# samiazirar/mvtracker

Hardware: AMD Instinct MI355X
Metric: query-points*frames/sec, 4-view 24-frame 512x512 @1024 queries (higher is better)
Workload: dtype bf16; 1 GPU; c3: 4-view synthetic 24-frame 512x512, 1024 queries, bf16 (configs[2], the metric's config); 4-view 24-frame 512x512, 1024 queries per GPU, corr K=16 x 4 levels, iters=4, 3 windows, random-init weights (seeded recipe); queries_total=1024, parallelism=query-shard x1, frame_store=bf16 rows

## Files before the change

### mvtracker_amd/csrc/conv_rows.hip

```cpp
#include <stdlib.h>

#include "common.h"

namespace {

typedef __bf16 bf16x8 __attribute__((ext_vector_type(8)));
typedef __bf16 bf16x4 __attribute__((ext_vector_type(4)));
typedef unsigned u32x4 __attribute__((ext_vector_type(4)));
typedef unsigned u32x2 __attribute__((ext_vector_type(2)));
typedef float f32x2 __attribute__((ext_vector_type(2)));
typedef short s16x2 __attribute__((ext_vector_type(2)));
typedef __bf16 bf16x2 __attribute__((ext_vector_type(2)));

#ifdef MVT_STAMPS
#ifndef MVT_STAMP_WG
#define MVT_STAMP_WG 2000
#endif
__device__ unsigned long long mvt_conv_stamp_buf[2 * 8 * 128];
#define CSTAMP(i)                                                                                                  \
  do {                                                                                                             \
    __builtin_amdgcn_sched_barrier(0);                                                                             \
    unsigned long long t_;                                                                                         \
    asm volatile("s_memtime %0\n\ts_waitcnt lgkmcnt(0)" : "=s"(t_)::"memory");                                     \
    __builtin_amdgcn_sched_barrier(0);                                                                             \
// ... 606 lines not shown

constexpr int SPR = 2 * TR + 5, SPC = 2 * TC + 6;
constexpr int SNP = SPR * SPC;
constexpr int SKW = 7 * 32;
constexpr int SLW = SKW + 8;

template <int TN, bool STAGED>
__global__ __launch_bounds__(256) void stem7x7_rows_bf16(RowsArgs p) {
  constexpr int TM = 2, BN = TN * 32;
  constexpr int NPL = (SNP + 255) / 256;
  constexpr int NWF = (BN * (SKW / 8) + 255) / 256;
  __shared__ __attribute__((aligned(16))) unsigned short Ps[SNP * 4];
  __shared__ __attribute__((aligned(16))) unsigned short Ws[BN * SLW];
  __shared__ float wst[TR * BN * 2];
  const int t = threadIdx.x;
  for (int i = t; i < TR * BN * 2; i += 256) wst[i] = 0.f;
  const int Ho = (p.H + 6 - 7) / 2 + 1, Wo = (p.W + 6 - 7) / 2 + 1;
  const int tiles_x = (Wo + TC - 1) / TC, tiles_y = (Ho + TR - 1) / TR;
  int b = blockIdx.x;
  const int tx = b % tiles_x; b /= tiles_x;
  const int ty = b % tiles_y;
  const long long img = b / tiles_y;
  const int y0 = ty * TR, x0 = tx * TC;
  const float* in = p.in + img * (long long)p.H * p.W * 4;
  const long long hw = (long long)p.H * p.W;
  long long plane0 = 0;
  if (p.rgb) {
    const long long gi = p.rgb_img0 + img;
    const long long tt = gi / p.rgb_V, vv = gi - tt * p.rgb_V;
    plane0 = ((vv * p.rgb_T + tt) * 3) * hw;
  }

  f32x4 rp[NPL];
#pragma unroll
  for (int i = 0; i < NPL; ++i) {
    const int f = t + 256 * i;
    const int py = f / SPC, px = f - py * SPC;
    const int gy = 2 * y0 - 3 + py, gx = 2 * x0 - 3 + px;
    const bool ok = f < SNP && (unsigned)gy < (unsigned)p.H && (unsigned)gx < (unsigned)p.W;
    const int cy = min(max(gy, 0), p.H - 1), cx = min(max(gx, 0), p.W - 1);
    f32x4 v;
    if (p.rgb) {
      const long long o = plane0 + (long long)cy * p.W + cx;
      float c0, c1, c2;
      if (p.rgb_u8) {
        const unsigned char* sp = static_cast<const unsigned char*>(p.rgb) + o;
        c0 = (float)sp[0]; c1 = (float)sp[hw]; c2 = (float)sp[2 * hw];
      } else {
        const float* sp = static_cast<const float*>(p.rgb) + o;
        c0 = sp[0]; c1 = sp[hw]; c2 = sp[2 * hw];
      }
      v = (f32x4){2.0f * (c0 / 255.0f) - 1.0f, 2.0f * (c1 / 255.0f) - 1.0f, 2.0f * (c2 / 255.0f) - 1.0f, 0.0f};
    } else {
      v = *reinterpret_cast<const f32x4*>(in + ((long long)cy * p.W + cx) * 4);
    }
    rp[i] = ok ? v : (f32x4){0.f, 0.f, 0.f, 0.f};
  }
  u32x4 rw[NWF];
#pragma unroll
  for (int i = 0; i < NWF; ++i) {
    const int u = t + 256 * i;
    const int n = u / (SKW / 8), part = u - n * (SKW / 8);
    rw[i] = *reinterpret_cast<const u32x4*>(p.w + (long long)min(n, p.Cout - 1) * p.ldw + part * 8);
    if (n >= p.Cout) rw[i] = (u32x4){0u, 0u, 0u, 0u};
  }
#pragma unroll
  for (int i = 0; i < NPL; ++i) {
    const int f = t + 256 * i;
    if (f < SNP) *reinterpret_cast<u32x2*>(&Ps[f * 4]) = __builtin_bit_cast(u32x2, __builtin_convertvector(rp[i], bf16x4));
  }
#pragma unroll
  for (int i = 0; i < NWF; ++i) {
    const int u = t + 256 * i;
    const int n = u / (SKW / 8), part = u - n * (SKW / 8);
    if (n < BN) *reinterpret_cast<u32x4*>(&Ws[n * SLW + part * 8]) = rw[i];
  }
  __syncthreads();

  const int lane = t & 63;
  const int wm = __builtin_amdgcn_readfirstlane(t >> 6);
  const int r = lane & 31, h = lane >> 5;
  const unsigned short* Pl = Ps + ((wm * TM * 2) * SPC + 2 * r + 2 * h) * 4;
  const unsigned short* Wl = Ws + r * SLW + h * 8;
  f32x16 acc[TM][TN];
#pragma unroll
  for (int i = 0; i < TM; ++i)
#pragma unroll
    for (int j = 0; j < TN; ++j)
#pragma unroll
      for (int e = 0; e < 16; ++e) acc[i][j][e] = 0.f;
#pragma unroll
  for (int kh = 0; kh < 7; ++kh) {
#pragma unroll
    for (int ks = 0; ks < 2; ++ks) {
      bf16x8 a[TM], bb[TN];
#pragma unroll
      for (int i = 0; i < TM; ++i) a[i] = __builtin_bit_cast(bf16x8, *reinterpret_cast<const u32x4*>(Pl + ((2 * i + kh) * SPC + 4 * ks) * 4));
#pragma unroll
      for (int j = 0; j < TN; ++j) bb[j] = __builtin_bit_cast(bf16x8, *reinterpret_cast<const u32x4*>(Wl + j * 32 * SLW + kh * 32 + ks * 16));
#pragma unroll
      for (int i = 0; i < TM; ++i)
#pragma unroll
        for (int j = 0; j < TN; ++j) acc[i][j] = __builtin_amdgcn_mfma_f32_32x32x16_bf16(a[i], bb[j], acc[i][j], 0, 0, 0);
    }
  }

  __syncthreads();
  static_assert(4 * stage_elems<TN>() <= BN * SLW, "staging tiles fit the weight buffer");
  epilogue_rows<TM, TN, true, STAGED>(acc, p, img, Ho, Wo, y0 + wm * TM, x0, 0, tiles_x, tx, lane, Ws + wm * stage_elems<TN>(), wst, wm * TM);
  if (p.out_part) {
    __syncthreads();
    write_tile_stats<TR, BN>(p, wst, img, ty * tiles_x + tx, 0, t);
  }
}


constexpr int BG_BN = 256;
constexpr int BG_PC = TC + 2;
constexpr int BG_PSLOTS = (TR + 2) * BG_PC;
constexpr int BG_PINSTR = 24;
constexpr int BG_PBYTES = BG_PINSTR * 1024;
constexpr int BG_PROW = BG_PC * 64;
constexpr int BG_WBYTES = 3 * BG_BN * 64;
constexpr int BG_WST = TR * BG_BN * 2 * 4;
constexpr int BG_LDS = 2 * BG_PBYTES + 2 * BG_WBYTES;
static_assert(BG_PSLOTS * 64 <= BG_PBYTES, "patch slots fit the buffer");
static_assert(BG_WBYTES / 1024 == 6 * 8, "six weight DMA wave-instructions per wave and stage");
static_assert(BG_LDS <= 160 * 1024 && BG_WST <= 2 * BG_WBYTES, "one workgroup per CU");
static_assert(8 * stage_elems<2>() * 2 <= 2 * BG_PBYTES, "the epilogue's staging tiles reuse the patch buffers");

__device__ __attribute__((aligned(64))) unsigned mvt_conv_zero_page[16];

typedef __attribute__((address_space(3))) void* lds_void_ptr;
typedef const __attribute__((address_space(1))) void* gbl_void_ptr;

__device__ __forceinline__ void dma16(const void* src, unsigned char* lds_dst_uniform) {
  const unsigned dst = __builtin_amdgcn_readfirstlane((unsigned)(uintptr_t)(lds_void_ptr)lds_dst_uniform);
  unsigned keep;
  asm volatile("s_mov_b32 %0, m0\n\ts_mov_b32 m0, %2\n\ts_nop 0\n\tglobal_load_lds_dwordx4 %1, off\n\ts_mov_b32 m0, %0"
               : "=&s"(keep)
               : "v"(src), "s"(dst)
               : "memory");
}

__global__ __launch_bounds__(512, 2) void conv3x3_big_bf16(RowsArgs p) {
  constexpr int TM = 4, TN = 2;
  __shared__ __attribute__((aligned(1024))) unsigned char lds[BG_LDS];
  unsigned char* const Pb = lds;
  unsigned char* const Wb = lds + 2 * BG_PBYTES;
  float* const wst = reinterpret_cast<float*>(Wb);

  const int t = threadIdx.x, lane = t & 63;
  const int wave = __builtin_amdgcn_readfirstlane(t >> 6);
  const int wm = wave & 1, wn = wave >> 1;
  const int r = lane & 31, h = lane >> 5;
  const int Ho = p.H, Wo = p.W;
  const int tiles_x = (Wo + TC - 1) / TC, tiles_y = (Ho + TR - 1) / TR;
  const int tiles_n = p.Cout / BG_BN;
  int b;
  {
    const unsigned nwg = gridDim.x, q = nwg / 8, rr = nwg % 8, xcd = blockIdx.x % 8;
    b = (int)((xcd < rr ? xcd * (q + 1) : rr * (q + 1) + (xcd - rr) * q) + blockIdx.x / 8);
  }
  const int tn = b % tiles_n; b /= tiles_n;
  const int tx = b % tiles_x; b /= tiles_x;
  const int ty = b % tiles_y;
  const long long img = b / tiles_y;
  const int y0 = ty * TR, x0 = tx * TC, n0 = tn * BG_BN;
  const unsigned char* const in_img = reinterpret_cast<const unsigned char*>(p.in) + img * (long long)p.H * p.W * p.Cin * 2;
  const unsigned char* const wbase = reinterpret_cast<const unsigned char*>(p.w);
  const unsigned char* const zero = reinterpret_cast<const unsigned char*>(mvt_conv_zero_page);

  int poff[3];
#pragma unroll
  for (int i = 0; i < 3; ++i) {
    const int P = (wave + 8 * i) * 64 + lane;
    const int slot = P >> 2, py = slot / BG_PC, px = slot - py * BG_PC;
    const int q = (P & 3) ^ ((px >> 2) & 3);
    const int gy = y0 - 1 + py, gx = x0 - 1 + px;
    const bool ok = slot < BG_PSLOTS && (unsigned)gy < (unsigned)p.H && (unsigned)gx < (unsigned)p.W;
    poff[i] = ok ? ((gy * p.W + gx) * p.Cin + q * 8) * 2 : -1;
  }
  int woff[6];
#pragma unroll
  for (int i = 0; i < 6; ++i) {
    const int R = (wave + 8 * i) * 16 + (lane >> 2);
    const int q = (lane & 3) ^ ((R >> 2) & 3);
    woff[i] = ((n0 + (R & 255)) * p.ldw + (R >> 8) * p.Cin + q * 8) * 2;
  }
  auto dma_weight = [&](int stage, int dst_stage, int i) {
    const int c = stage / 3, kh = stage - 3 * c;
    dma16(wbase + ((long long)kh * 3 * p.Cin + c * CK) * 2 + woff[i], Wb + (dst_stage & 1) * BG_WBYTES + wave * 1024 + i * 8192);
  };
  auto dma_patch1 = [&](int c, int dst_c, int i) {
    dma16(poff[i] >= 0 ? in_img + c * CK * 2 + poff[i] : zero, Pb + (dst_c & 1) * BG_PBYTES + wave * 1024 + i * 8192);
  };

  const int nchunk = p.Cin / CK;
#pragma unroll
  for (int i = 0; i < 3; ++i) dma_patch1(0, 0, i);
#pragma unroll
  for (int i = 0; i < 6; ++i) dma_weight(0, 0, i);

  int pa[3][2], wl[2];
#pragma unroll
  for (int kw = 0; kw < 3; ++kw)
#pragma unroll
    for (int ks = 0; ks < 2; ++ks)
      pa[kw][ks] = (TM * wm * BG_PC + kw + r) * 64 + (((2 * ks + h) ^ (((kw + r) >> 2) & 3)) << 4);
#pragma unroll
  for (int ks = 0; ks < 2; ++ks) wl[ks] = (64 * wn + r) * 64 + (((2 * ks + h) ^ ((r >> 2) & 3)) << 4);

  f32x16 acc[TM][TN];
#pragma unroll
  for (int i = 0; i < TM; ++i)
#pragma unroll
    for (int j = 0; j < TN; ++j)
#pragma unroll
      for (int e = 0; e < 16; ++e) acc[i][j][e] = 0.f;

  bf16x8 a[2][TM], bb[2][TN];
  auto read_group = [&](int set, int g, int kh, const unsigned char* Pc, const unsigned char* Wc) {
    const int kw = g >> 1, ks = g & 1;
#pragma unroll
    for (int i = 0; i < TM; ++i)
      a[set][i] = __builtin_bit_cast(bf16x8, *reinterpret_cast<const u32x4*>(Pc + pa[kw][ks] + (i + kh) * BG_PROW));
#pragma unroll
    for (int j = 0; j < TN; ++j)
      bb[set][j] = __builtin_bit_cast(bf16x8, *reinterpret_cast<const u32x4*>(Wc + wl[ks] + kw * (BG_BN * 64) + j * 2048));
  };
  auto mfma_group = [&](int set) {
#pragma unroll
    for (int i = 0; i < TM; ++i)
#pragma unroll
      for (int j = 0; j < TN; ++j) acc[i][j] = __builtin_amdgcn_mfma_f32_32x32x16_bf16(a[set][i], bb[set][j], acc[i][j], 0, 0, 0);
  };
  CSTAMP(0);
#ifdef MVT_BIG_PRIO
  if (wave >= 4) __builtin_amdgcn_s_setprio(1);
#endif
  asm volatile("s_waitcnt vmcnt(0)" ::: "memory");
  __builtin_amdgcn_s_barrier();
  read_group(0, 0, 0, Pb, Wb);
  for (int c = 0; c < nchunk; ++c) {
    const unsigned char* const Pc = Pb + (c & 1) * BG_PBYTES;
#pragma unroll
    for (int kh = 0; kh < 3; ++kh) {
      const int stage = 3 * c + kh;
      const int stage_n = stage + 1 < 3 * nchunk ? stage + 1 : stage, chunk_n = c + 1 < nchunk ? c + 1 : c;
      const unsigned char* const Wc = Wb + (stage & 1) * BG_WBYTES;
#pragma unroll
      for (int g = 0; g < 5; ++g) {
        read_group((g + 1) & 1, g + 1, kh, Pc, Wc);
#ifdef MVT_BIG_EARLY
        if (g == 0) {
#pragma unroll
          for (int i = 0; i < 6; ++i) dma_weight(stage_n, stage + 1, i);
        } else if (g == 1 && kh == 0) {
#pragma unroll
          for (int i = 0; i < 3; ++i) dma_patch1(chunk_n, c + 1, i);
        }
#else
        if (g < 3) {
          dma_weight(stage_n, stage + 1, 2 * g);
          dma_weight(stage_n, stage + 1, 2 * g + 1);
        } else if (kh == 0) {
          dma_patch1(chunk_n, c + 1, g == 3 ? 0 : 2);
          if (g == 3) dma_patch1(chunk_n, c + 1, 1);
        }
#endif
        __builtin_amdgcn_sched_barrier(0);
        mfma_group(g & 1);
        __builtin_amdgcn_sched_barrier(0);
        if (stage < 12) CSTAMP(1 + 10 * stage + g);
      }
      if (kh == 0) asm volatile("s_waitcnt vmcnt(3) lgkmcnt(0)" ::: "memory");
      else asm volatile("s_waitcnt vmcnt(0) lgkmcnt(0)" ::: "memory");
      if (stage < 12) CSTAMP(1 + 10 * stage + 5);
      __builtin_amdgcn_s_barrier();
      if (stage < 12) CSTAMP(1 + 10 * stage + 6);
      read_group(0, 0, kh == 2 ? 0 : kh + 1, kh == 2 ? Pb + ((c + 1) & 1) * BG_PBYTES : Pc, Wb + ((stage + 1) & 1) * BG_WBYTES);
      __builtin_amdgcn_sched_barrier(0);
      mfma_group(1);
      __builtin_amdgcn_sched_barrier(0);
      if (stage < 12) CSTAMP(1 + 10 * stage + 7);
    }
  }
  CSTAMP(124);
  asm volatile("s_waitcnt vmcnt(0)" ::: "memory");
  __builtin_amdgcn_s_barrier();
  for (int i = lane; i < TM * 64 * 2; i += 64) wst[((wm * TM + (i >> 7)) * BG_BN + wn * 64) * 2 + (i & 127)] = 0.f;

  epilogue_rows<TM, TN, false, true, BG_BN>(acc, p, img, Ho, Wo, y0 + wm * TM, x0, n0 + wn * 64, tiles_x, tx, lane,
                                             reinterpret_cast<unsigned short*>(Pb) + wave * stage_elems<TN>(), wst + wn * 64 * 2, wm * TM);
  CSTAMP(125);
  if (p.out_part) {
    __syncthreads();
    write_tile_stats<TR, BG_BN>(p, wst, img, ty * tiles_x + tx, n0, t);
  }
  CSTAMP(126);
}


}

#ifdef MVT_STAMPS
extern "C" int mvt_debug_read_conv_stamps(unsigned long long* host) {
  return hipMemcpyFromSymbol(host, HIP_SYMBOL(mvt_conv_stamp_buf), sizeof(unsigned long long) * 2 * 8 * 128) == hipSuccess ? MVT_OK : MVT_ERR_HIP_BASE;
}
extern "C" int mvt_debug_clear_conv_stamps() {
  static unsigned long long z[2 * 8 * 128];
  return hipMemcpyToSymbol(HIP_SYMBOL(mvt_conv_stamp_buf), z, sizeof(z)) == hipSuccess ? MVT_OK : MVT_ERR_HIP_BASE;
}
#endif

static int rows_nw8() {
  static const int v = getenv("MVT_ROWS_NW8") ? atoi(getenv("MVT_ROWS_NW8")) : 0;
  return v;
}
__attribute__((visibility("hidden"))) int mvt_detail_conv_rows_tile_rows(int ksize, int stride, int Ho) {
  if (ksize == 3 && stride == 1) return (rows_nw8() == 1 && Ho % 16 == 0) ? 16 : (rows_nw8() == 2 ? 4 : 8);
  if (ksize == 3) return 4;
  if (ksize == 7) return TR;
  return 8;
}
__attribute__((visibility("hidden"))) int mvt_detail_conv_rows_slots(int Ho, int Wo, int tile_rows) {
  return (int)(mvt_cdiv(Ho, tile_rows) * mvt_cdiv(Wo, TC));
}

__attribute__((visibility("hidden"))) int mvt_detail_conv_rows(const void* in, const unsigned short* w, int ldw, const float* bias, void* out,
                                                               int n, int H, int W, int Cin, int Cout, int ksize, int stride, int ldo,
                                                               int io_flags, const float* in_stats, float* out_partial,
                                                               hipStream_t stream) {
  MVT_REQUIRE((ksize == 1 || ksize == 3) && (stride == 1 || stride == 2));
  MVT_REQUIRE((!in_stats || Cin <= MAXC) && Cin % CK == 0 && (long long)H * W * Cin < (1LL << 31) && (long long)Cout * ldw < (1LL << 31));
  MVT_REQUIRE((long long)(TC + 8) * ldo * 4 < (1LL << 31));
  const int pad = ksize == 3 ? 1 : 0;
  const int Ho = (H + 2 * pad - ksize) / stride + 1, Wo = (W + 2 * pad - ksize) / stride + 1;
  RowsArgs a{};
  a.in = (const float*)in; a.w = w; a.bias = bias; a.out = (float*)out; a.in_stats = in_stats; a.out_part = out_partial;
  a.H = H; a.W = W; a.Cin = Cin; a.Cout = Cout; a.ldw = ldw; a.ldo = ldo;
  a.slots = mvt_detail_conv_rows_slots(Ho, Wo, mvt_detail_conv_rows_tile_rows(ksize, stride, Ho));
  a.in_bf16 = io_flags & MVT_IO_IN_BF16 ? 1 : 0;
  a.out_bf16 = io_flags & MVT_IO_OUT_BF16 ? 1 : 0;
  const bool n96 = Cout % 64 != 0 && Cout % 96 == 0;
  const int bn = n96 ? 96 : 64;
  const bool st_ok = a.out_bf16 && Cout % 8 == 0 && ldo % 8 == 0 && ((uintptr_t)out & 15) == 0;
#define LAUNCH2(TM_, TN_, KS_, S_, NW_, INB_)                                                                                       \
  do {                                                                                                                             \
    constexpr bool fits = NW_ * stage_elems<TN_>() <= Geo<TM_, KS_, S_, NW_>::NSLOT * LDP;                                          \
    if (fits && st_ok) hipLaunchKernelGGL((conv_rows_bf16<TM_, TN_, KS_, S_, INB_, NW_, fits>), grid, dim3(64 * NW_), 0, stream, a); \
    else hipLaunchKernelGGL((conv_rows_bf16<TM_, TN_, KS_, S_, INB_, NW_, false>), grid, dim3(64 * NW_), 0, stream, a);            \
  } while (0)
#define LAUNCH(TM_, KS_, S_, NW_)                                                                                                   \
  do {                                                                                                                             \
    const long long tiles = (long long)n * mvt_cdiv(Ho, NW_ * TM_) * mvt_cdiv(Wo, TC) * mvt_cdiv(Cout, bn);                        \
    MVT_REQUIRE(tiles < (1LL << 31));                                                                                              \
    const dim3 grid((unsigned)tiles);                                                                                              \
    if (n96) {                                                                                                                     \
      if (a.in_bf16) LAUNCH2(TM_, 3, KS_, S_, NW_, true);                                                                          \
      else LAUNCH2(TM_, 3, KS_, S_, NW_, false);                                                                                   \
    } else {                                                                                                                       \
      if (a.in_bf16) LAUNCH2(TM_, 2, KS_, S_, NW_, true);                                                                          \
      else LAUNCH2(TM_, 2, KS_, S_, NW_, false);                                                                                   \
    }                                                                                                                              \
  } while (0)
  const int nw8 = rows_nw8();
  if (ksize == 3 && stride == 1 && !in_stats && !(io_flags & MVT_IO_SHORT_WG) && a.in_bf16 && st_ok && Cout % BG_BN == 0 && ((uintptr_t)in & 15) == 0 && Cin % 8 == 0 &&
      ldw % 8 == 0 && ((uintptr_t)w & 15) == 0 && (long long)Cout * ldw * 2 < (1LL << 31) && (long long)H * W * Cin * 2 < (1LL << 31)) {
    const char* e = getenv("MVT_CONV_BIG");
    if (!e || atoi(e) != 0) {
      const long long tiles = (long long)n * mvt_cdiv(Ho, TR) * mvt_cdiv(Wo, TC) * (Cout / BG_BN);
      MVT_REQUIRE(tiles < (1LL << 31));
      hipLaunchKernelGGL(conv3x3_big_bf16, dim3((unsigned)tiles), dim3(512), 0, stream, a);
      return mvt_launch_status();
    }
  }
  if (ksize == 3 && stride == 1 && nw8 == 1 && Ho % 16 == 0) LAUNCH(2, 3, 1, 8);
  else if (ksize == 3 && stride == 1 && nw8 == 2) LAUNCH(1, 3, 1, 4);
  else if (ksize == 3 && stride == 1) LAUNCH(2, 3, 1, 4);
  else if (ksize == 3) LAUNCH(1, 3, 2, 4);
  else if (stride == 1) LAUNCH(2, 1, 1, 4);
  else LAUNCH(2, 1, 2, 4);
#undef LAUNCH2
#undef LAUNCH
  return mvt_launch_status();
}

__attribute__((visibility("hidden"))) int mvt_detail_conv3x3s2_down(const void* in, const unsigned short* w3, int ldw3, const float* b3,
                                                                    const unsigned short* wd, int ldwd, const float* bd, void* out3,
                                                                    void* outd, int n, int H, int W, int Cin, int Cout, int ldo,
                                                                    float* part3, float* partd, hipStream_t stream) {
  MVT_REQUIRE(in && w3 && wd && out3 && outd && n > 0 && Cin % CK == 0 && Cout % 32 == 0 && Cout % 8 == 0 && ldo % 8 == 0 && ldo >= Cout);
  MVT_REQUIRE((long long)H * W * Cin < (1LL << 31) && (long long)Cout * ldw3 < (1LL << 31) && ldwd >= Cin && ldw3 >= 9 * Cin);
  MVT_REQUIRE(((uintptr_t)in & 15) == 0 && ((uintptr_t)out3 & 15) == 0 && ((uintptr_t)outd & 15) == 0 && ((uintptr_t)w3 & 15) == 0 &&
              ((uintptr_t)wd & 15) == 0 && ldw3 % 8 == 0 && ldwd % 8 == 0 && (!part3) == (!partd));
  const int Ho = (H + 2 - 3) / 2 + 1, Wo = (W + 2 - 3) / 2 + 1;
  RowsArgs a{};
  a.in = (const float*)in; a.w = w3; a.bias = b3; a.out = (float*)out3; a.in_stats = nullptr; a.out_part = part3;
  a.H = H; a.W = W; a.Cin = Cin; a.Cout = Cout; a.ldw = ldw3; a.ldo = ldo;
  a.slots = mvt_detail_conv_rows_slots(Ho, Wo, 4);
  a.in_bf16 = 1; a.out_bf16 = 1;
  a.w2 = wd; a.bias2 = bd; a.out2 = (float*)outd; a.out_part2 = partd; a.ldw2 = ldwd;
  const bool n96 = Cout % 64 != 0 && Cout % 96 == 0;
  const long long tiles = (long long)n * mvt_cdiv(Ho, 4) * mvt_cdiv(Wo, TC) * mvt_cdiv(Cout, n96 ? 96 : 64);
  MVT_REQUIRE(tiles < (1LL << 31));
  static_assert(4 * stage_elems<2>() <= Geo<1, 3, 2, 4>::NSLOT * LDP && 4 * stage_elems<3>() <= Geo<1, 3, 2, 4>::NSLOT * LDP, "staged epilogue");
  if (n96) hipLaunchKernelGGL((conv_rows_bf16<1, 3, 3, 2, true, 4, true, true>), dim3((unsigned)tiles), dim3(256), 0, stream, a);
  else hipLaunchKernelGGL((conv_rows_bf16<1, 2, 3, 2, true, 4, true, true>), dim3((unsigned)tiles), dim3(256), 0, stream, a);
  return mvt_launch_status();
}

__attribute__((visibility("hidden"))) int mvt_detail_stem7x7_rows_src(const float* in, const void* rgb, int rgb_u8, int rgb_V, int rgb_T,
                                                                      long long rgb_img0, const unsigned short* w, int ldw,
                                                                      const float* bias, void* out, int n, int H, int W, int Cout, int ldo,
                                                                      int io_flags, float* out_partial, hipStream_t stream);
__attribute__((visibility("hidden"))) int mvt_detail_stem7x7_rows(const float* in, const unsigned short* w, int ldw, const float* bias,
                                                                  void* out, int n, int H, int W, int Cout, int ldo, int io_flags,
                                                                  float* out_partial, hipStream_t stream) {
  return mvt_detail_stem7x7_rows_src(in, nullptr, 0, 0, 0, 0, w, ldw, bias, out, n, H, W, Cout, ldo, io_flags, out_partial, stream);
}
__attribute__((visibility("hidden"))) int mvt_detail_stem7x7_rows_src(const float* in, const void* rgb, int rgb_u8, int rgb_V, int rgb_T,
                                                                      long long rgb_img0, const unsigned short* w, int ldw,
                                                                      const float* bias, void* out, int n, int H, int W, int Cout, int ldo,
                                                                      int io_flags, float* out_partial, hipStream_t stream) {
  MVT_REQUIRE(Cout > 0 && Cout <= 64 && ldw >= SKW && (long long)H * W * 4 < (1LL << 31) && !(io_flags & MVT_IO_IN_BF16));
  MVT_REQUIRE((in != nullptr) != (rgb != nullptr));
  MVT_REQUIRE(!rgb || (rgb_V > 0 && rgb_T > 0 && rgb_img0 >= 0 && rgb_img0 + n <= (long long)rgb_V * rgb_T && (rgb_u8 == 0 || rgb_u8 == 1)));
  const int Ho = (H - 1) / 2 + 1, Wo = (W - 1) / 2 + 1;
  RowsArgs a{};
  a.rgb = rgb; a.rgb_u8 = rgb_u8; a.rgb_V = rgb_V; a.rgb_T = rgb_T; a.rgb_img0 = rgb_img0;
  a.in = in; a.w = w; a.bias = bias; a.out = (float*)out; a.in_stats = nullptr; a.out_part = out_partial;
  a.H = H; a.W = W; a.Cin = 4; a.Cout = Cout; a.ldw = ldw; a.ldo = ldo;
  a.slots = mvt_detail_conv_rows_slots(Ho, Wo, TR);
  a.in_bf16 = 0;
  a.out_bf16 = io_flags & MVT_IO_OUT_BF16 ? 1 : 0;
  const long long tiles = (long long)n * mvt_cdiv(Ho, TR) * mvt_cdiv(Wo, TC);
  MVT_REQUIRE(tiles < (1LL << 31) && (long long)(TC + 8) * ldo * 4 < (1LL << 31));
  const bool st_ok = a.out_bf16 && Cout % 8 == 0 && ldo % 8 == 0 && ((uintptr_t)out & 15) == 0;
  if (Cout <= 32) {
    if (st_ok) hipLaunchKernelGGL((stem7x7_rows_bf16<1, true>), dim3((unsigned)tiles), dim3(256), 0, stream, a);
    else hipLaunchKernelGGL((stem7x7_rows_bf16<1, false>), dim3((unsigned)tiles), dim3(256), 0, stream, a);
  } else {
    if (st_ok) hipLaunchKernelGGL((stem7x7_rows_bf16<2, true>), dim3((unsigned)tiles), dim3(256), 0, stream, a);
    else hipLaunchKernelGGL((stem7x7_rows_bf16<2, false>), dim3((unsigned)tiles), dim3(256), 0, stream, a);
  }
  return mvt_launch_status();
}
```

Baseline: 1.020 million query-points*frames/s.

## Add four-workgroup-per-CU 3x3 conv kernel for normalized or small-channel rows

Adds a new 256-thread 3x3 stride-1 bf16 convolution kernel sized to fit four workgroups per CU in LDS. It fuses input normalization/ReLU from per-image stats into the patch store, register-prefetches the next weight row and patch chunk, and remaps block ids across XCDs. It is dispatched for cases the big kernel rejects (for example in_stats present) when there are enough tiles. It also stops caching the env var lookup, which adds a getenv per call.

```diff
diff --git a/mvtracker_amd/csrc/conv_rows.hip b/mvtracker_amd/csrc/conv_rows.hip
--- a/mvtracker_amd/csrc/conv_rows.hip
+++ b/mvtracker_amd/csrc/conv_rows.hip
@@ -932,6 +932,169 @@
 }
 
 
+constexpr int W4_BN = 64;
+constexpr int W4_PC = TC + 2;
+constexpr int W4_NSLOT = (TR + 2) * W4_PC;
+constexpr int W4_PBYTES = W4_NSLOT * LDP * 2;
+constexpr int W4_WBYTES = 3 * W4_BN * 64;
+constexpr int W4_MAXC = 128;
+constexpr int W4_NPL = (W4_NSLOT * 4 + 255) / 256;
+static_assert(W4_PBYTES + W4_WBYTES + 2 * W4_MAXC * 4 <= 40 * 1024, "four workgroups per CU");
+static_assert(TR * W4_BN * 2 * 4 <= W4_WBYTES, "the statistics table reuses the weight buffer");
+static_assert(4 * stage_elems<2>() * 2 <= W4_PBYTES, "the epilogue's staging tiles reuse the patch");
+
+__global__ __launch_bounds__(256, 4) void conv3x3_wg4_bf16(RowsArgs p) {
+  constexpr int TM = 2, TN = 2, BN = W4_BN;
+  __shared__ __attribute__((aligned(16))) unsigned char Pb[W4_PBYTES];
+  __shared__ __attribute__((aligned(16))) unsigned char Wb[W4_WBYTES];
+  __shared__ __attribute__((aligned(16))) float Sst[2 * W4_MAXC];
+  float* const wst = reinterpret_cast<float*>(Wb);
+
+  const int t = threadIdx.x;
+  const int Ho = p.H, Wo = p.W;
+  const int tiles_x = (Wo + TC - 1) / TC, tiles_y = (Ho + TR - 1) / TR;
+  const int tiles_n = p.Cout / BN;
+  int b;
+  {
+    const unsigned nwg = gridDim.x, q = nwg / 8, rr = nwg % 8, xcd = blockIdx.x % 8;
+    b = (int)((xcd < rr ? xcd * (q + 1) : rr * (q + 1) + (xcd - rr) * q) + blockIdx.x / 8);
+  }
+  const int tn = b % tiles_n; b /= tiles_n;
+  const int tx = b % tiles_x; b /= tiles_x;
+  const int ty = b % tiles_y;
+  const long long img = b / tiles_y;
+  const int y0 = ty * TR, x0 = tx * TC, n0 = tn * BN;
+  const char* const in_img = reinterpret_cast<const char*>(reinterpret_cast<const unsigned short*>(p.in) + img * (long long)p.H * p.W * p.Cin);
+
+  auto tid = [&]() {
+    int v;
+    asm volatile("v_mov_b32 %0, %1" : "=v"(v) : "v"(threadIdx.x));
+    return v;
+  };
+  u32x4 rp[W4_NPL];
+  u32x4 rw[3];
+  auto load_patch = [&](int c0) {
+    const int tt = tid();
+    const char* base = in_img + c0 * 2;
+#pragma unroll
+    for (int i = 0; i < W4_NPL; ++i) {
+      const int sl = (tt + 256 * i) >> 2;
+      const int py = sl / W4_PC, px = sl - py * W4_PC;
+      const int cy = min(max(y0 - 1 + py, 0), p.H - 1), cx = min(max(x0 - 1 + px, 0), p.W - 1);
+      rp[i] = *reinterpret_cast<const u32x4*>(base + (unsigned)(((cy * p.W + cx) * p.Cin + (tt & 3) * 8) * 2));
+    }
+  };
+  auto store_patch = [&](int c0) {
+    const int tt = tid(), q = tt & 3;
+    auto pair = [](unsigned ww, float nm0, float nm1, float r0, float r1) -> unsigned {
+      f32x2 v = (f32x2){__uint_as_float(ww << 16), __uint_as_float(ww & 0xFFFF0000u)};
+      v = (v + (f32x2){nm0, nm1}) * (f32x2){r0, r1};
+      s16x2 h2 = __builtin_bit_cast(s16x2, __builtin_convertvector(v, bf16x2));
+      h2 = __builtin_elementwise_max(h2, (s16x2){0, 0});
+      return __builtin_bit_cast(unsigned, h2);
+    };
+    if (p.in_stats) {
+#pragma unroll
+      for (int half = 0; half < 2; ++half) {
+        const float* sp = &Sst[(c0 + q * 8 + 4 * half) * 2];
+        const f32x4 a = *reinterpret_cast<const f32x4*>(sp), b4 = *reinterpret_cast<const f32x4*>(sp + 4);
+#pragma unroll
+        for (int i = 0; i < W4_NPL; ++i) {
+          rp[i][2 * half] = pair(rp[i][2 * half], -a[0], -a[2], a[1], a[3]);
+          rp[i][2 * half + 1] = pair(rp[i][2 * half + 1], -b4[0], -b4[2], b4[1], b4[3]);
+        }
+      }
+    }
+#pragma unroll
+    for (int i = 0; i < W4_NPL; ++i) {
+      const int sl = (tt + 256 * i) >> 2;
+      if (sl >= W4_NSLOT) continue;
+      const int py = sl / W4_PC, px = sl - py * W4_PC;
+      const int gy = y0 - 1 + py, gx = x0 - 1 + px;
+      const bool ok = (unsigned)gy < (unsigned)p.H && (unsigned)gx < (unsigned)p.W;
+      *reinterpret_cast<u32x4*>(Pb + sl * (LDP * 2) + q * 16) = ok ? rp[i] : (u32x4){0u, 0u, 0u, 0u};
+    }
+  };
+  auto load_w = [&](int c0, int kh) {
+    const int tt = tid();
+    const unsigned wg = ((n0 + (tt >> 2)) * p.ldw + (tt & 3) * 8) * 2;
+    const char* base = reinterpret_cast<const char*>(p.w + kh * 3 * p.Cin + c0);
+#pragma unroll
+    for (int i = 0; i < 3; ++i) rw[i] = *reinterpret_cast<const u32x4*>(base + i * p.Cin * 2 + wg);
+  };
+  auto store_w = [&]() {
+    const int tt = tid();
+    const int wdst = (tt >> 2) * 64 + (((tt & 3) ^ ((tt >> 4) & 3)) << 4);
+#pragma unroll
+    for (int i = 0; i < 3; ++i) *reinterpret_cast<u32x4*>(Wb + i * 4096 + wdst) = rw[i];
+  };
+
+  load_patch(0);
+  load_w(0, 0);
+  if (p.in_stats) {
+    for (int i = t; i < 2 * p.Cin; i += 256) Sst[i] = p.in_stats[img * 2 * p.Cin + i];
+    __syncthreads();
+  }
+  const int lane = t & 63;
+  const int wm = __builtin_amdgcn_readfirstlane(t >> 6);
+  const int r = lane & 31, h = lane >> 5;
+  const unsigned char* const Pl = Pb + ((TM * wm * W4_PC + r) * LDP + h * 8) * 2;
+  int wl[2];
+#pragma unroll
+  for (int ks = 0; ks < 2; ++ks) wl[ks] = r * 64 + (((2 * ks + h) ^ ((r >> 2) & 3)) << 4);
+
+  f32x16 acc[TM][TN];
+#pragma unroll
+  for (int i = 0; i < TM; ++i)
+#pragma unroll
+    for (int j = 0; j < TN; ++j)
+#pragma unroll
+      for (int e = 0; e < 16; ++e) acc[i][j][e] = 0.f;
+
+  const int nchunk = p.Cin / CK;
+  for (int c = 0; c < nchunk; ++c) {
+    const bool more = c + 1 < nchunk;
+#pragma unroll
+    for (int kh = 0; kh < 3; ++kh) {
+      store_w();
+      if (kh == 0) store_patch(c * CK);
+      __syncthreads();
+      if (kh + 1 < 3) {
+        load_w(c * CK, kh + 1);
+      } else if (more) {
+        load_w((c + 1) * CK, 0);
+        load_patch((c + 1) * CK);
+      }
+#pragma unroll
+      for (int kw = 0; kw < 3; ++kw) {
+#pragma unroll
+        for (int ks = 0; ks < CK / 16; ++ks) {
+          bf16x8 a[TM], bb[TN];
+#pragma unroll
+          for (int i = 0; i < TM; ++i)
+            a[i] = __builtin_bit_cast(bf16x8, *reinterpret_cast<const u32x4*>(Pl + (((i + kh) * W4_PC + kw) * LDP + ks * 16) * 2));
+#pragma unroll
+          for (int j = 0; j < TN; ++j) bb[j] = __builtin_bit_cast(bf16x8, *reinterpret_cast<const u32x4*>(Wb + wl[ks] + (kw * BN + j * 32) * 64));
+#pragma unroll
+          for (int i = 0; i < TM; ++i)
+#pragma unroll
+            for (int j = 0; j < TN; ++j) acc[i][j] = __builtin_amdgcn_mfma_f32_32x32x16_bf16(a[i], bb[j], acc[i][j], 0, 0, 0);
+        }
+      }
+      __syncthreads();
+    }
+  }
+
+  for (int i = tid() & 63; i < TM * BN * 2; i += 64) wst[wm * TM * BN * 2 + i] = 0.f;
+  epilogue_rows<TM, TN, false, true>(acc, p, img, Ho, Wo, y0 + wm * TM, x0, n0, tiles_x, tx, tid() & 63,
+                                     reinterpret_cast<unsigned short*>(Pb) + wm * stage_elems<TN>(), wst, wm * TM);
+  if (p.out_part) {
+    __syncthreads();
+    write_tile_stats<TR, BN>(p, wst, img, ty * tiles_x + tx, n0, tid());
+  }
+}
+
+
 }
 
 #ifdef MVT_STAMPS
@@ -945,8 +1108,8 @@
 #endif
 
 static int rows_nw8() {
-  static const int v = getenv("MVT_ROWS_NW8") ? atoi(getenv("MVT_ROWS_NW8")) : 0;
-  return v;
+  const char* e = getenv("MVT_ROWS_NW8");
+  return e ? atoi(e) : 0;
 }
 __attribute__((visibility("hidden"))) int mvt_detail_conv_rows_tile_rows(int ksize, int stride, int Ho) {
   if (ksize == 3 && stride == 1) return (rows_nw8() == 1 && Ho % 16 == 0) ? 16 : (rows_nw8() == 2 ? 4 : 8);
@@ -970,7 +1133,8 @@
   RowsArgs a{};
   a.in = (const float*)in; a.w = w; a.bias = bias; a.out = (float*)out; a.in_stats = in_stats; a.out_part = out_partial;
   a.H = H; a.W = W; a.Cin = Cin; a.Cout = Cout; a.ldw = ldw; a.ldo = ldo;
-  a.slots = mvt_detail_conv_rows_slots(Ho, Wo, mvt_detail_conv_rows_tile_rows(ksize, stride, Ho));
+  const int tile_rows = mvt_detail_conv_rows_tile_rows(ksize, stride, Ho);
+  a.slots = mvt_detail_conv_rows_slots(Ho, Wo, tile_rows);
   a.in_bf16 = io_flags & MVT_IO_IN_BF16 ? 1 : 0;
   a.out_bf16 = io_flags & MVT_IO_OUT_BF16 ? 1 : 0;
   const bool n96 = Cout % 64 != 0 && Cout % 96 == 0;
@@ -996,13 +1160,23 @@
     }                                                                                                                              \
   } while (0)
   const int nw8 = rows_nw8();
-  if (ksize == 3 && stride == 1 && !in_stats && !(io_flags & MVT_IO_SHORT_WG) && a.in_bf16 && st_ok && Cout % BG_BN == 0 && ((uintptr_t)in & 15) == 0 && Cin % 8 == 0 &&
+  if (ksize == 3 && stride == 1 && tile_rows == TR && !in_stats && !(io_flags & MVT_IO_SHORT_WG) && a.in_bf16 && st_ok && Cout % BG_BN == 0 && ((uintptr_t)in & 15) == 0 && Cin % 8 == 0 &&
       ldw % 8 == 0 && ((uintptr_t)w & 15) == 0 && (long long)Cout * ldw * 2 < (1LL << 31) && (long long)H * W * Cin * 2 < (1LL << 31)) {
     const char* e = getenv("MVT_CONV_BIG");
     if (!e || atoi(e) != 0) {
       const long long tiles = (long long)n * mvt_cdiv(Ho, TR) * mvt_cdiv(Wo, TC) * (Cout / BG_BN);
       MVT_REQUIRE(tiles < (1LL << 31));
       hipLaunchKernelGGL(conv3x3_big_bf16, dim3((unsigned)tiles), dim3(512), 0, stream, a);
+      return mvt_launch_status();
+    }
+  }
+  if (ksize == 3 && stride == 1 && tile_rows == TR && a.in_bf16 && st_ok && Cout % W4_BN == 0 && (!in_stats || Cin <= W4_MAXC) &&
+      (long long)n * mvt_cdiv(Ho, TR) * mvt_cdiv(Wo, TC) * (Cout / W4_BN) >= 4 * 256) {
+    const char* e = getenv("MVT_ROWS_WG4");
+    if (!e || atoi(e) != 0) {
+      const long long tiles = (long long)n * mvt_cdiv(Ho, TR) * mvt_cdiv(Wo, TC) * (Cout / W4_BN);
+      MVT_REQUIRE(tiles < (1LL << 31));
+      hipLaunchKernelGGL(conv3x3_wg4_bf16, dim3((unsigned)tiles), dim3(256), 0, stream, a);
       return mvt_launch_status();
     }
   }
```

Result: no change. 1.029 million query-points*frames/s, median of 6 (+0.9%).
